# sunnyHelen/JPerceiver

Hardware: AMD Instinct MI355X
Metric: train images/sec (full train step, synthetic 3-frame batches) (higher is better)
Workload: dtype f32

## Files before the change

### include/jperceiver_hip.h

```cpp
#ifndef JPERCEIVER_HIP_H
#define JPERCEIVER_HIP_H
#include <stdint.h>

#ifdef __cplusplus
extern "C" {
#endif

int jp_conv2d_fwd(const float* x, const float* w, const float* bias, float* y, int N, int Cin, int H, int W, int Cout, int KH, int stride, int pad, int pad_mode, int act, float* ws, int ws_state, float* split_ws, const float* amax_x, float* amax_y, int* amax_y_done, float* amax_ws, float* bn_stats, int* bn_stats_parts, void* stream);
int jp_conv2d_fwd_src3(const float* x0, int c0, int up0, const float* x1, int c1, int up1, const float* x2, int c2, int up2, const float* w, const float* bias, float* y, int N, int H, int W, int Cout, int KH, int stride, int pad, int pad_mode, int act, float* ws, int ws_state, float* split_ws, const float* amax_x0, const float* amax_x1, const float* amax_x2, float* amax_y, int* amax_y_done, float* amax_ws, float* bn_stats, int* bn_stats_parts, void* stream);
int jp_conv2d_dgrad(const float* dy, const float* w, float* dx, int N, int Cin, int H, int W, int Cout, int KH, int stride, int pad, int pad_mode, int accumulate, float* ws, int ws_state, float* split_ws, const float* amax_dy, float* amax_dx, int* amax_dx_done, float* amax_ws, void* stream);
int jp_conv2d_dgrad_src3(const float* dy, const float* w, float* dx0, int c0, int up0, int acc0, float* dx1, int c1, int up1, int acc1, float* dx2, int c2, int up2, int acc2, int N, int H, int W, int Cout, int KH, int stride, int pad, int pad_mode, float* ws, int ws_state, float* split_ws, const float* amax_dy, float* amax_dx0, int* amax_dx0_done, float* amax_ws, void* stream);
long jp_conv2d_dgrad_src3_split_floats(int c0, int up0, int c1, int up1, int c2, int up2, int N, int H, int W);
int jp_conv2d_dgrad_src3_ok(int c0, int up0, int c1, int up1, int c2, int up2, int N, int H, int W, int Cout, int KH, int stride, int pad, int pad_mode);
int jp_conv2d_up_head_ok(int c0, int up0, int c1, int c2, int Cout, int KH, int stride, int pad, int pad_mode, int H, int W);
int jp_conv2d_wgrad(const float* x, const float* dy, float* dw, int N, int Cin, int H, int W, int Cout, int KH, int stride, int pad, int pad_mode, int accumulate, float* ws, long ws_floats, const float* amax_x, const float* amax_dy, float* amax_ws, void* stream);
int jp_conv2d_wgrad_src3(const float* x0, int c0, int up0, const float* x1, int c1, int up1, const float* x2, int c2, int up2, const float* dy, float* dw, int N, int H, int W, int Cout, int KH, int stride, int pad, int pad_mode, int accumulate, float* ws, long ws_floats, const float* amax_x0, const float* amax_x1, const float* amax_x2, const float* amax_dy, float* amax_ws, void* stream);
long jp_conv2d_ws_floats(int Cin, int Cout, int KH, int which);
long jp_conv2d_fwd_bn_stats_floats(int N, int OH, int OW, int Cout);
long jp_conv2d_fwd_split_floats(int N, int Cin, int H, int W, int Cout, int KH, int stride, int pad);
long jp_conv2d_dgrad_split_floats(int N, int Cin, int H, int W, int Cout, int KH, int stride, int pad);
long jp_conv2d_wgrad_ws_floats(int N, int Cin, int H, int W, int Cout, int KH, int stride, int pad);
long jp_conv2d_wgrad_src3_ws_floats(int c0, int up0, int c1, int up1, int c2, int up2, int N, int H, int W, int Cout, int KH, int stride, int pad, int pad_mode);
long jp_channel_sum_ws_floats(int N, int C, int HW);
int jp_channel_sum(const float* x, float* out, int N, int C, int HW, int accumulate, float* ws, void* stream);
// ... 12 lines not shown
long jp_bn_ws_doubles(int N, int C, int HW);
int jp_bn_train_fwd(const float* x, const float* gamma, const float* beta, const float* residual, float* y, float* running_mean, float* running_var, float* save_mean, float* save_invstd, double* ws, int N, int C, int HW, float momentum, float eps, int relu, int n_updates, float* amax_y, const float* conv_stats, int conv_parts, void* stream);
int jp_bn_train_bwd(const float* dy, const float* x, const float* y, const float* gamma, const float* beta, const float* save_mean, const float* save_invstd, float* dx, float* dres, float* dgamma, float* dbeta, double* ws, int N, int C, int HW, int relu, int acc_param_grads, float* amax_dx, void* stream);
int jp_bn_eval_fwd(const float* x, const float* gamma, const float* beta, const float* running_mean, const float* running_var, const float* residual, float* y, int N, int C, int HW, float eps, int relu, void* stream);
int jp_bn_relu_pool_fwd(const float* x, const float* gamma, const float* beta, float* pooled, uint8_t* idx, float* running_mean, float* running_var, float* save_mean, float* save_invstd, double* ws, int N, int C, int H, int W, float momentum, float eps, int n_updates, float* amax_y, void* stream);
long jp_bn_relu_pool_bwd_ws_doubles(int N, int C, int H, int W);
int jp_bn_relu_pool_bwd(const float* dpool, const uint8_t* idx, const float* x, const float* gamma, const float* beta, const float* save_mean, const float* save_invstd, float* dx, float* dgamma, float* dbeta, double* ws, int N, int C, int H, int W, int acc_param_grads, void* stream);

int jp_bn_fold_conv(const float* w, const float* conv_bias, const float* gamma, const float* beta, const float* running_mean, const float* running_var, float eps, float* w_out, float* bias_out, int Cout, int K, void* stream);
int jp_add_relu(const float* a, const float* b, float* out, long n, int relu, float* amax_out, void* stream);

int jp_maxpool_fwd(const float* x, float* y, uint8_t* idx, int NC, int H, int W, int k, int s, int p, void* stream);
int jp_maxpool_bwd(const float* dy, const uint8_t* idx, float* dx, const float* addend, int NC, int H, int W, int k, int s, int p, float* amax_dx, void* stream);
int jp_upsample2x_fwd(const float* x, float* y, int N, int C, int H, int W, int dstC, int dc0, void* stream);
int jp_upsample2x_bwd(const float* dy, float* dx, int N, int C, int H, int W, int Ctot, int c0, int accumulate, void* stream);
int jp_copy_channels(const float* src, float* dst, int N, int C, int HW, int srcC, int sc0, int dstC, int dc0, int accumulate, void* stream);
int jp_axpby(const float* a, const float* b, float* out, long n, float alpha, float beta, void* stream);
int jp_sum_n(const float* a0, const float* a1, const float* a2, const float* a3, const float* a4, float* out, long n, float* amax_out, void* stream);
int jp_mul(const float* a, const float* b, float* out, long n, float scale, void* stream);
int jp_affine(const float* a, float* out, long n, float scale, float shift, void* stream);
int jp_act_fwd(const float* x, float* y, long n, int act, void* stream);
int jp_act_bwd(const float* dy, const float* y, float* dx, long n, int act, float* amax_dx, void* stream);
long jp_act_bwd_bias_ws_floats(int N, int C, int HW);
int jp_act_bwd_bias(const float* dy, const float* y, float* dx, float* dbias, int N, int C, int HW, int act, float* amax_dx, float* bias_ws, void* stream);
int jp_mul_bcast_c(const float* a, const float* s, float* out, int N, int C, int HW, void* stream);
int jp_mul_bcast_c_bwd_s(const float* dout, const float* a, float* ds, int N, int C, int HW, void* stream);
int jp_bilinear_fwd(const float* x, float* y, int NC, int H, int W, int OH, int OW, void* stream);
int jp_bilinear_bwd(const float* dy, float* dx, int NC, int H, int W, int OH, int OW, int accumulate, void* stream);
int jp_area_downsample(const float* x, float* y, int NC, int H, int W, int f, void* stream);
int jp_fill(float* out, long n, float v, void* stream);
int jp_warp_perspective(const float* src, const float* Hm, float* dst, int B, int h, int w, int OH, int OW, void* stream);
int jp_softmax_c2(const float* x, float* y, int N, int HW, void* stream);
int jp_disp_to_depth(const float* disp, float* depth, long n, float min_depth, float max_depth, void* stream);
int jp_scale_label_assemble(const float* zwarp, const float* laywarp, const uint8_t* polymask, float* out, int B, int H, int W, int mode, void* stream);
int jp_fill_convex_poly(const int* pts, int npts, uint8_t* mask, int H, int W, void* stream);

int jp_gemm_strided_batched(const float* A, const float* B, float* C, int M, int N, int K, int lda, int ldb, int ldc, long strideA, long strideB, long strideC, int batch, int transA, int transB, float alpha, float beta, void* stream);
int jp_bias_act_rows(float* y, const float* bias, int M, int N, int act, void* stream);
int jp_colsum(const float* x, float* out, int M, int N, int accumulate, void* stream);
int jp_colmax(const float* E, float* val, int64_t* arg, int B, int R, int Cn, void* stream);
int jp_colmax_bwd(const float* dval, const int64_t* arg, float* dE, int B, int R, int Cn, void* stream);
int jp_gather_cols(const float* V, const int64_t* arg, float* T, int B, int C, int Nn, void* stream);
int jp_gather_cols_bwd(const float* dT, const int64_t* arg, float* dV, int B, int C, int Nn, void* stream);
int jp_spatial_mean(const float* x, float* out, int BC, int HW, float scale, void* stream);
int jp_spatial_mean_bwd(const float* dout, float* dx, int BC, int HW, float scale, void* stream);
int jp_bcast_matmul_fwd(const float* attn, const float* V, float* out, int B, int C, int n, void* stream);
int jp_bcast_matmul_bwd(const float* attn, const float* V, const float* dOut, float* dattn, float* dV, int B, int C, int n, void* stream);
int jp_ratio_finalize(const double* acc, float* out, double scale, void* stream);

int jp_pose_fwd(const float* axisangle, const float* translation, const float* K, float* T, float* P, int B, int invert, void* stream);
int jp_pose_bwd(const double* dP, const float* axisangle, const float* translation, const float* K, float* daxisangle, float* dtranslation, int B, int invert, int accumulate, void* stream);
int jp_cgt_warp_fwd(const float* disp, int hs, int ws, const float* invK, const float* P, const float* color, float* pred, int B, int H, int W, float min_depth, float max_depth, void* stream);
int jp_cgt_warp_bwd(const float* dpred, const float* disp, int hs, int ws, const float* invK, const float* P, const float* color, float* ddisp_up, double* dP, int B, int H, int W, float min_depth, float max_depth, int accumulate, void* stream);
int jp_ssim_l1_fwd(const float* pred, const float* target, float* out, int B, int H, int W, void* stream);
int jp_ssim_l1_bwd(const float* pred, const float* target, const int64_t* min_index, int cand, const float* gout, float gscale, float* dpred, int B, int H, int W, void* stream);
int jp_minreproj_fwd(const float* c0, const float* c1, const float* c2, const float* c3, const float* noise0, const float* noise1, int64_t* min_index, double* acc, long total, void* stream);
int jp_scalar_finalize(const double* in, float* out, int n, double scale, void* stream);
int jp_ssim_map(const float* x, const float* y, float* out, int NC, int H, int W, void* stream);
int jp_backproject(const float* depth, const float* invK, float* out, int B, int H, int W, void* stream);
int jp_project(const float* points, const float* K, const float* T, float* out, int B, int H, int W, float eps, void* stream);

int jp_row_sum(const float* x, double* out, int rows, int cols, void* stream);
int jp_smooth_fwd(const float* disp, const double* dsum, const float* img, double* acc, int B, int h, int w, void* stream);
int jp_smooth_bwd(const float* disp, const double* dsum, const float* img, const float* gout, float scale, float* g, double* gd, float* ddisp, int B, int h, int w, int accumulate, void* stream);
int jp_scale_loss_fwd(const float* disp, int hs, int ws, const float* label, double* acc, int B, int FH, int FW, float min_depth, float max_depth, int y_lo, int y_hi, int x_lo, int x_hi, void* stream);
int jp_scale_loss_bwd(const float* disp, int hs, int ws, const float* label, const double* acc, const float* gout, float scale, float* ddisp, int B, int FH, int FW, float min_depth, float max_depth, int y_lo, int y_hi, int x_lo, int x_hi, int accumulate, void* stream);
int jp_layout_loss_fwd(const float* logits, const float* label, const float* sdf, double* sums, float* loss, int B, int h, int w, float w0, float w1, float lw, float cew, float l2w, float ra, float ralpha, float rbeta, void* stream);
int jp_layout_loss_bwd(const float* logits, const float* label, const float* sdf, const double* sums, const float* gout, float* dlogits, int B, int h, int w, float w0, float w1, float lw, float cew, float l2w, float ra, float ralpha, float rbeta, int accumulate, void* stream);
int jp_sdf(const float* label, float* sdf, int* ws, int B, int h, int w, void* stream);
int jp_l1_fwd(const float* a, const float* b, double* acc, long n, void* stream);
int jp_l1_bwd(const float* a, const float* b, const float* gout, float scale, float* da, float* db, long n, void* stream);

int jp_sumsq_blocks(void);
int jp_grad_sumsq_partials(const float* g, double* partials, long n, void* stream);
int jp_sum_doubles(const double* in, double* out, int count, void* stream);
int jp_adam_clip_step(float* p, const float* g, float* m, float* v, long n, const double* normsq, float grad_scale, float max_norm, double lr, double beta1, double beta2, double eps, int step, void* stream);
int jp_adam_clip_step_dev(float* p, const float* g, float* m, float* v, long n, const double* normsq, float grad_scale, float max_norm, double beta1, double beta2, double eps, const float* state, void* stream);
int jp_rng_keep_mask(float* out, long n, uint64_t seed, float p_drop, void* stream);
int jp_rng_normal(float* out, long n, uint64_t seed, void* stream);
int jp_rng_keep_mask_dev(float* out, long n, const long* base, long offset, float p_drop, void* stream);
int jp_rng_normal_dev(float* out, long n, const long* base, long offset, void* stream);

int jp_confusion2(const float* logits, const float* gt, double* counts, int B, int HW, void* stream);
int jp_depth_eval_prepare(const float* disp_resized, const float* gt, float* pred, uint8_t* valid, int H, int W, int y0, int y1, int x0, int x1, float dmin, float dmax, void* stream);
int jp_masked_median(const float* x, const uint8_t* valid, int n, float* out, void* stream);
int jp_depth_errors(const float* gt, const float* pred, const uint8_t* valid, int n, const float* med_gt, const float* med_pred, float fixed_scale, float dmin, float dmax, double* sums, void* stream);

long jp_depth_eval_batch_ws_bytes(int B, int H, int W);
int jp_depth_eval_batch(const float* disp, const float* gt, int B, int h, int w, int H, int W, int y0, int y1, int x0, int x1, float mask_min, float mask_max, double min_depth, double max_depth, float fixed_scale, double* sums, float* med, void* ws, void* stream);
long jp_lidar_depth_ws_bytes(int B, int H, int W);
int jp_lidar_depth_map(const float* pts, const long long* offsets, const double* P, const unsigned char* flip, int B, int H, int W, int vel_depth, double* out64, float* out32, void* ws, void* stream);

int jp_disp_resize_depth(const float* disp, float* depth_out, float* disp_out, int B, int h, int w, int OH, int OW, double min_depth, double max_depth, void* stream);
long jp_quantiles_ws_bytes(int rows);
int jp_quantiles(const float* x, int rows, int n, const float* q, int nq, float* out, void* ws, void* stream);
int jp_colorize_u8(const float* x, int rows, int n, const float* vmin_vmax, const uint8_t* lut, uint8_t* out, void* stream);
int jp_layout_classes_u8(const float* road_logits, const float* car_logits, uint8_t* cls, uint8_t* rgb, int B, int HW, void* stream);

int jp_stream_pose_pair(const float* frame, float* ring, const int* count, float* pair, float* amax_out, int B, int H, int W, void* stream);
int jp_stream_traj_push(const float* T, double* pose, double* traj, int* count, int B, int capacity, void* stream);

int jp_bev_fuse(const uint8_t* layout, const double* pose, int pose_stride, int N, int* counts, int B, int occ, double res_f, double off, double max_range, int Mh, int Mw, double res, double org_r, double org_c, void* stream);
int jp_bev_map_classes(const int* counts, uint8_t* cls, uint8_t* rgb, int B, int cells, double min_seen, double road_frac, double car_frac, void* stream);
int jp_bev_map_mark(uint8_t* rgb, int B, int Mh, int Mw, const double* traj, int n, int capacity, double res, double org_r, double org_c, int color, void* stream);

int jp_depth_bev_lift(const float* depth, const double* cam, int* grid, int B, int H, int W, int occ, double res_f, double off, double min_range, double max_range, double h_min, double h_max, double obst_h, int accumulate, void* stream);
int jp_depth_bev_classes(const int* grid, uint8_t* cls, float* height, int B, int cells, int min_points, int obst_points, void* stream);
int jp_bev_agree(const uint8_t* lifted, const uint8_t* layout, int* out, int B, int cells, void* stream);
// ... 38 lines not shown
```

### jperceiver_amd/csrc/photometric.hip

```cpp
#include "jp_common.h"
#include <algorithm>

namespace {

constexpr int TPB = 256;
constexpr float SSIM_C1 = 0.0001f, SSIM_C2 = 0.0009f;

__device__ void rodrigues(const float v[3], float R[9]) {
    const float th = sqrtf(v[0] * v[0] + v[1] * v[1] + v[2] * v[2]);
    const float inv = 1.f / (th + 1e-7f);
    const float x = v[0] * inv, y = v[1] * inv, z = v[2] * inv;
    const float ca = cosf(th), sa = sinf(th), C = 1.f - ca;
    R[0] = x * x * C + ca;     R[1] = x * y * C - z * sa; R[2] = z * x * C + y * sa;
    R[3] = x * y * C + z * sa; R[4] = y * y * C + ca;     R[5] = y * z * C - x * sa;
    R[6] = z * x * C - y * sa; R[7] = y * z * C + x * sa; R[8] = z * z * C + ca;
}

__global__ void pose_fwd_kernel(const float* __restrict__ aa, const float* __restrict__ tr,
                                const float* __restrict__ K, float* __restrict__ T, float* __restrict__ P, int B,
                                int invert) {
    const int b = blockIdx.x * blockDim.x + threadIdx.x;
    if (b >= B) return;
    float v[3] = {aa[3 * b], aa[3 * b + 1], aa[3 * b + 2]};
    float t[3] = {tr[3 * b], tr[3 * b + 1], tr[3 * b + 2]};
// ... 183 lines not shown
    for (int it = 0; it < CGT_PPT; ++it) {
        const int p = (blockIdx.x * CGT_PPT + it) * TPB + threadIdx.x;
        if (p >= H * W) break;
        const int y = p / W, x = p - y * W;
        const float* Pb = Pm + 12 * b;
        const WarpGeo g = warp_geo(disp + (size_t)b * hs * ws, hs, ws, invK + 16 * b, Pb, y, x, H, W, min_disp,
                                   max_disp, (float)hs / (float)H, (float)ws / (float)W);
        const int x0 = (int)floorf(g.ix), y0 = (int)floorf(g.iy);
        const float tx = g.ix - (float)x0, ty = g.iy - (float)y0;
        const bool xin = x0 + 1 <= W - 1, yin = y0 + 1 <= H - 1;
        const int x1 = xin ? x0 + 1 : x0, y1 = yin ? y0 + 1 : y0;
        const size_t HW = (size_t)H * W;
        const float* c = color + (size_t)b * 3 * HW;
        float gix = 0.f, giy = 0.f;
#pragma unroll
        for (int ch = 0; ch < 3; ++ch) {
            const float* cc = c + ch * HW;
            const float go = dpred[((size_t)b * 3 + ch) * HW + p];
            const float v00 = cc[y0 * W + x0];
            const float v01 = xin ? cc[y0 * W + x1] : 0.f;
            const float v10 = yin ? cc[y1 * W + x0] : 0.f;
            const float v11 = (xin && yin) ? cc[y1 * W + x1] : 0.f;
            gix += go * (-(v00 * (1.f - ty)) + v01 * (1.f - ty) - v10 * ty + v11 * ty);
            giy += go * (-(v00 * (1.f - tx)) - v01 * tx + v10 * (1.f - tx) + v11 * tx);
        }
        const float du = gix * g.mx * (0.5f * (float)W) * (2.f / (float)(W - 1));
        const float dv = giy * g.my * (0.5f * (float)H) * (2.f / (float)(H - 1));
        const float zi = g.pz + 1e-7f;
        const float dpx = du / zi, dpy = dv / zi;
        const float dpz = -(du * g.px + dv * g.py) / (zi * zi);
        const float X = g.depth * g.rx, Y = g.depth * g.ry, Z = g.depth * g.rz;
        dPl[0] += dpx * X; dPl[1] += dpx * Y; dPl[2] += dpx * Z; dPl[3] += dpx;
        dPl[4] += dpy * X; dPl[5] += dpy * Y; dPl[6] += dpy * Z; dPl[7] += dpy;
        dPl[8] += dpz * X; dPl[9] += dpz * Y; dPl[10] += dpz * Z; dPl[11] += dpz;
        const float dX = Pb[0] * dpx + Pb[4] * dpy + Pb[8] * dpz;
        const float dY = Pb[1] * dpx + Pb[5] * dpy + Pb[9] * dpz;
        const float dZ = Pb[2] * dpx + Pb[6] * dpy + Pb[10] * dpz;
        const float ddepth = dX * g.rx + dY * g.ry + dZ * g.rz;
        const float dd = -(max_disp - min_disp) * g.depth * g.depth * ddepth;
        float* q = ddisp_up + (size_t)b * HW + p;
        *q = accumulate ? *q + dd : dd;
    }
    const int lane = threadIdx.x & 63, wv = threadIdx.x >> 6;
#pragma unroll
    for (int i = 0; i < 12; ++i) {
        const float s = jp_wave_sum(dPl[i]);
        if (lane == 0) red[i][wv] = s;
    }
    __syncthreads();
    if (threadIdx.x < 12) {
        const double s = (double)red[threadIdx.x][0] + red[threadIdx.x][1] + red[threadIdx.x][2] + red[threadIdx.x][3];
        atomicAdd(&dP[12 * b + threadIdx.x], s);
    }
}

constexpr int SSIM_ROWS = 4;

struct RowSums { float x, y, xx, yy, xy; };

__device__ __forceinline__ RowSums ssim_hsum(const float* __restrict__ xr, const float* __restrict__ yr, int il, int ic,
                                             int ir, float& xc, float& yc) {
    const float xl = xr[il], xrn = xr[ir], yl = yr[il], yrn = yr[ir];
    xc = xr[ic];
    yc = yr[ic];
    RowSums s;
    s.x = xl + xc + xrn;
    s.y = yl + yc + yrn;
    s.xx = xl * xl + xc * xc + xrn * xrn;
    s.yy = yl * yl + yc * yc + yrn * yrn;
    s.xy = xl * yl + xc * yc + xrn * yrn;
    return s;
}

__global__ __launch_bounds__(TPB) void ssim_l1_fwd_kernel(const float* __restrict__ pred,
                                                          const float* __restrict__ target,
                                                          float* __restrict__ out, int H, int W) {
    const int lane = threadIdx.x & 63, wv = threadIdx.x >> 6;
    const int x = (blockIdx.x * 4 + wv) * 64 + lane;
    if ((blockIdx.x * 4 + wv) * 64 >= W) return;
    const int b = blockIdx.z;
    const int ybeg = blockIdx.y * SSIM_ROWS, yend = min(H, ybeg + SSIM_ROWS);
    const size_t HW = (size_t)H * W;
    const int ic = min(x, W - 1), il = jp_reflect(ic - 1, W), ir = jp_reflect(ic + 1, W);
    float accS[SSIM_ROWS], accL[SSIM_ROWS];
#pragma unroll
    for (int r = 0; r < SSIM_ROWS; ++r) accS[r] = accL[r] = 0.f;
#pragma unroll
    for (int ch = 0; ch < 3; ++ch) {
        const float* xp = pred + ((size_t)b * 3 + ch) * HW;
        const float* yp = target + ((size_t)b * 3 + ch) * HW;
        RowSums r0, r1, r2;
        float xc, yc, xc1, yc1;
        {
            const size_t oa = (size_t)jp_reflect(ybeg - 1, H) * W, ob = (size_t)ybeg * W;
            r0 = ssim_hsum(xp + oa, yp + oa, il, ic, ir, xc, yc);
            r1 = ssim_hsum(xp + ob, yp + ob, il, ic, ir, xc1, yc1);
        }
#pragma unroll
        for (int r = 0; r < SSIM_ROWS; ++r) {
            const int y = min(ybeg + r, H - 1);
            const size_t on = (size_t)jp_reflect(y + 1, H) * W;
            float xc2, yc2;
            r2 = ssim_hsum(xp + on, yp + on, il, ic, ir, xc2, yc2);
            const float k = 1.f / 9.f;
            const float mx = (r0.x + r1.x + r2.x) * k, my = (r0.y + r1.y + r2.y) * k;
            const float sx = (r0.xx + r1.xx + r2.xx) * k - mx * mx;
// ... 63 lines not shown
            const float xl = nxl, xr = nxr, yl = nyl, yr = nyr;
            xc2 = nxc; yc2 = nyc;
            const int miv = nmi;
            if (t + 1 < SSIMB_ROWS + 2) {
                on = rowoff(t + 1);
                nxl = xp[on + il]; nxc = xp[on + ic]; nxr = xp[on + ir];
                nyl = yp[on + il]; nyc = yp[on + ic]; nyr = yp[on + ir];
                if (mi32) nmi = mi32[2 * ((size_t)qrow(t + 1) * W + ic)];
            }
            r2.x = xl + xc2 + xr;
            r2.y = yl + yc2 + yr;
            r2.xx = xl * xl + xc2 * xc2 + xr * xr;
            r2.yy = yl * yl + yc2 * yc2 + yr * yr;
            r2.xy = xl * yl + xc2 * yc2 + xr * yr;
            const bool q_in = q >= 0 && q < H && col_in;
            const float g = (q_in && miv == cand) ? gs : 0.f;
            const float k = 1.f / 9.f;
            const float mx = (r0.x + r1.x + r2.x) * k, my = (r0.y + r1.y + r2.y) * k;
            const float vx = (r0.xx + r1.xx + r2.xx) * k - mx * mx, vy = (r0.yy + r1.yy + r2.yy) * k - my * my;
            const float cxy = (r0.xy + r1.xy + r2.xy) * k - mx * my;
            const float n1 = 2.f * mx * my + SSIM_C1, n2 = 2.f * cxy + SSIM_C2;
            const float d1 = mx * mx + my * my + SSIM_C1, d2 = vx + vy + SSIM_C2;
            const float n = n1 * n2, d = d1 * d2;
            const float invd = 1.f / d, nd = n * invd;
            const float val = (1.f - nd) * 0.5f;
            const float gk = (val >= 0.f && val <= 1.f) ? g * (2.f / 9.f) : 0.f;
            const float G = gk * n1 * invd;
            const float Bc = -gk * nd * d1 * invd;
            const float A = gk * (my * (n2 - n1) * invd - nd * mx * (d2 - d1) * invd);
            const float hA2 = wl * __shfl_up(A, 1, 64) + A + wr * __shfl_down(A, 1, 64);
            const float hB2 = wl * __shfl_up(Bc, 1, 64) + Bc + wr * __shfl_down(Bc, 1, 64);
            const float hG2 = wl * __shfl_up(G, 1, 64) + G + wr * __shfl_down(G, 1, 64);
            if (t >= 2) {
                const int ry = q - 1;
                if (ry < yend && col_out) {
                    const float wu = (ry == 1) ? 2.f : 1.f, wd = (ry == H - 2) ? 2.f : 1.f;
                    const float SA = wu * hA0 + hA1 + wd * hA2;
                    const float SB = wu * hB0 + hB1 + wd * hB2;
                    const float SG = wu * hG0 + hG1 + wd * hG2;
                    const float df = xo - yo;
                    const float l1 = go * df * rsqrtf(df * df + 1e-6f);
                    dp[(size_t)ry * W + cq] = -0.5f * (0.85f / 3.f) * (SA + xo * SB + yo * SG) + (0.15f / 3.f) * l1;
                }
            }
            xo = xc1; yo = yc1; go = g;
            hA0 = hA1; hB0 = hB1; hG0 = hG1;
            hA1 = hA2; hB1 = hB2; hG1 = hG2;
            r0 = r1; r1 = r2;
            xc1 = xc2; yc1 = yc2;
        }
    }
}

__global__ __launch_bounds__(TPB) void minreproj_kernel(const float* __restrict__ c0, const float* __restrict__ c1,
                                                        const float* __restrict__ c2, const float* __restrict__ c3,
                                                        const float* __restrict__ n0, const float* __restrict__ n1,
                                                        int64_t* __restrict__ idx, double* __restrict__ acc,
                                                        long total) {
    __shared__ double sm[4];
    double s = 0.0;
    for (long i = (long)blockIdx.x * TPB + threadIdx.x; i < total; i += (long)gridDim.x * TPB) {
        float best = c0[i] + (n0 ? n0[i] * 1e-5f : 0.f);
        int bi = 0;
        if (c1) { const float v = c1[i] + (n1 ? n1[i] * 1e-5f : 0.f); if (v < best) { best = v; bi = 1; } }
        if (c2) { const float v = c2[i]; if (v < best) { best = v; bi = 2; } }
        if (c3) { const float v = c3[i]; if (v < best) { best = v; bi = 3; } }
        idx[i] = bi;
        s += (double)best;
    }
    s = jp_block_sum_d(s, sm);
    if (threadIdx.x == 0) atomicAdd(acc, s);
}

__global__ void scalar_finalize_kernel(const double* __restrict__ in, float* __restrict__ out, int n,
                                       double scale) {
    const int i = blockIdx.x * blockDim.x + threadIdx.x;
    if (i < n) out[i] = (float)(in[i] * scale);
}

__global__ __launch_bounds__(TPB) void ssim_map_kernel(const float* __restrict__ x, const float* __restrict__ y,
                                                       float* __restrict__ out, long total, int H, int W) {
    for (long i = (long)blockIdx.x * TPB + threadIdx.x; i < total; i += (long)gridDim.x * TPB) {
        const int px = (int)(i % W);
        const long t = i / W;
        const int py = (int)(t % H);
        const long plane = (t / H) * (long)H * W;
        float sx = 0.f, sy = 0.f, sxx = 0.f, syy = 0.f, sxy = 0.f;
#pragma unroll
        for (int dy = -1; dy <= 1; ++dy) {
            const int yy = jp_reflect(py + dy, H);
#pragma unroll
            for (int dx = -1; dx <= 1; ++dx) {
                const int xx = jp_reflect(px + dx, W);
                const float a = x[plane + (long)yy * W + xx], b = y[plane + (long)yy * W + xx];
                sx += a; sy += b; sxx += a * a; syy += b * b; sxy += a * b;
            }
        }
        const float k = 1.f / 9.f;
        const float mx = sx * k, my = sy * k;
        const float vx = sxx * k - mx * mx, vy = syy * k - my * my, cxy = sxy * k - mx * my;
        const float n = (2.f * mx * my + SSIM_C1) * (2.f * cxy + SSIM_C2);
        const float d = (mx * mx + my * my + SSIM_C1) * (vx + vy + SSIM_C2);
        out[i] = fminf(fmaxf((1.f - n / d) * 0.5f, 0.f), 1.f);
    }
}

// ... 31 lines not shown
                P[4 * r + c] = k[4 * r] * t[c] + k[4 * r + 1] * t[4 + c] + k[4 * r + 2] * t[8 + c] + k[4 * r + 3] * t[12 + c];
        const float* q = pts + (long)b * 4 * HW + p;
        const float X = q[0], Y = q[HW], Z = q[2 * HW], Wc = q[3 * HW];
        const float cx = P[0] * X + P[1] * Y + P[2] * Z + P[3] * Wc;
        const float cy = P[4] * X + P[5] * Y + P[6] * Z + P[7] * Wc;
        const float cz = P[8] * X + P[9] * Y + P[10] * Z + P[11] * Wc;
        const float inv = 1.f / (cz + eps);
        out[2 * i] = (cx * inv / (float)(W - 1) - 0.5f) * 2.f;
        out[2 * i + 1] = (cy * inv / (float)(H - 1) - 0.5f) * 2.f;
    }
}

}

#define JP_ST hipStream_t st = (hipStream_t)stream

extern "C" int jp_pose_fwd(const float* axisangle, const float* translation, const float* K, float* T, float* P,
                           int B, int invert, void* stream) {
    JP_CHECK_ARG(axisangle && translation && K && T && P && B > 0, "pose_fwd: bad args");
    JP_ST;
    hipLaunchKernelGGL(pose_fwd_kernel, dim3(jp_cdiv(B, 64)), dim3(64), 0, st, axisangle, translation, K, T, P, B, invert);
    JP_LAUNCH_CHECK();
}

extern "C" int jp_pose_bwd(const double* dP, const float* axisangle, const float* translation, const float* K,
                           float* daxisangle, float* dtranslation, int B, int invert, int accumulate, void* stream) {
    JP_CHECK_ARG(dP && axisangle && translation && K && daxisangle && dtranslation && B > 0, "pose_bwd: bad args");
    JP_ST;
    hipLaunchKernelGGL(pose_bwd_kernel, dim3(jp_cdiv(B, 64)), dim3(64), 0, st, dP, axisangle, translation, K,
                       daxisangle, dtranslation, B, invert, accumulate);
    JP_LAUNCH_CHECK();
}

extern "C" int jp_cgt_warp_fwd(const float* disp, int hs, int ws, const float* invK, const float* P,
                               const float* color, float* pred, int B, int H, int W, float min_depth,
                               float max_depth, void* stream) {
    JP_CHECK_ARG(disp && invK && P && color && pred && B > 0 && H > 1 && W > 1, "cgt_warp_fwd: bad args");
    JP_ST;
    hipLaunchKernelGGL(cgt_warp_fwd_kernel, dim3(jp_cdiv(W, TPB), B, jp_cdiv(H, CGT_FROWS)), dim3(TPB), 0, st, disp, hs, ws, invK, P,
                       color, pred, H, W, 1.f / max_depth, 1.f / min_depth);
    JP_LAUNCH_CHECK();
}

extern "C" int jp_cgt_warp_bwd(const float* dpred, const float* disp, int hs, int ws, const float* invK,
                               const float* P, const float* color, float* ddisp_up, double* dP, int B, int H, int W,
                               float min_depth, float max_depth, int accumulate, void* stream) {
    JP_CHECK_ARG(dpred && disp && invK && P && color && ddisp_up && dP && B > 0, "cgt_warp_bwd: bad args");
    JP_ST;
    hipLaunchKernelGGL(cgt_warp_bwd_kernel, dim3(jp_cdiv((long)H * W, TPB * CGT_PPT), B), dim3(TPB), 0, st, dpred, disp, hs, ws,
                       invK, P, color, ddisp_up, dP, H, W, 1.f / max_depth, 1.f / min_depth, accumulate);
    JP_LAUNCH_CHECK();
}

extern "C" int jp_ssim_l1_fwd(const float* pred, const float* target, float* out, int B, int H, int W,
                              void* stream) {
    JP_CHECK_ARG(pred && target && out && B > 0 && H >= 2 && W >= 2, "ssim_l1_fwd: bad args");
    JP_ST;
    dim3 grid(jp_cdiv(W, 256), jp_cdiv(H, SSIM_ROWS), B);
    hipLaunchKernelGGL(ssim_l1_fwd_kernel, grid, dim3(TPB), 0, st, pred, target, out, H, W);
    JP_LAUNCH_CHECK();
}

extern "C" int jp_ssim_l1_bwd(const float* pred, const float* target, const int64_t* min_index, int cand,
                              const float* gout, float gscale, float* dpred, int B, int H, int W, void* stream) {
    JP_CHECK_ARG(pred && target && dpred && B > 0 && H >= 2 && W >= 2, "ssim_l1_bwd: bad args");
    JP_ST;
    dim3 grid(jp_cdiv(jp_cdiv(W, 62), 4), jp_cdiv(H, SSIMB_ROWS), B);
    hipLaunchKernelGGL(ssim_l1_bwd_kernel, grid, dim3(TPB), 0, st, pred, target, min_index, cand, gout, gscale, dpred,
                       H, W);
    JP_LAUNCH_CHECK();
}

extern "C" int jp_minreproj_fwd(const float* c0, const float* c1, const float* c2, const float* c3,
                                const float* noise0, const float* noise1, int64_t* min_index, double* acc,
                                long total, void* stream) {
    JP_CHECK_ARG(c0 && min_index && acc && total > 0, "minreproj_fwd: bad args");
    JP_ST;
    JP_HIP(hipMemsetAsync(acc, 0, sizeof(double), st));
    hipLaunchKernelGGL(minreproj_kernel, dim3((int)std::min<long>((total + TPB - 1) / TPB, 2048)), dim3(TPB), 0, st,
                       c0, c1, c2, c3, noise0, noise1, min_index, acc, total);
    JP_LAUNCH_CHECK();
}

extern "C" int jp_scalar_finalize(const double* in, float* out, int n, double scale, void* stream) {
    JP_CHECK_ARG(in && out && n > 0, "scalar_finalize: bad args");
    JP_ST;
    hipLaunchKernelGGL(scalar_finalize_kernel, dim3(jp_cdiv(n, 64)), dim3(64), 0, st, in, out, n, scale);
    JP_LAUNCH_CHECK();
}

extern "C" int jp_ssim_map(const float* x, const float* y, float* out, int NC, int H, int W, void* stream) {
    JP_CHECK_ARG(x && y && out && NC > 0 && H >= 2 && W >= 2, "ssim_map: bad args");
    JP_ST;
    const long total = (long)NC * H * W;
    hipLaunchKernelGGL(ssim_map_kernel, dim3((int)std::min<long>((total + TPB - 1) / TPB, 65535)), dim3(TPB), 0, st, x, y, out,
                       total, H, W);
    JP_LAUNCH_CHECK();
}

extern "C" int jp_backproject(const float* depth, const float* invK, float* out, int B, int H, int W, void* stream) {
    JP_CHECK_ARG(depth && invK && out && B > 0 && H > 0 && W > 0, "backproject: bad args");
    JP_ST;
    const long total = (long)B * H * W;
    hipLaunchKernelGGL(backproject_kernel, dim3((int)std::min<long>((total + TPB - 1) / TPB, 65535)), dim3(TPB), 0, st, depth,
                       invK, out, B, H, W);
    JP_LAUNCH_CHECK();
// ... 12 lines not shown
```

### jperceiver_amd/ops_loss.py

```python
from __future__ import annotations

import torch

from ._lib import call
from . import ops
from .ops import Var, _rec, _new, gemm


def bmm_tn(k: Var, q: Var) -> Var:
    B, C, N = k.t.shape
    e = _new((B, N, N), k.t)
    gemm(k.t, q.t, e, N, N, C, N, N, N, C * N, C * N, N * N, B, tA=1)
    out = Var(e, k.rg or q.rg)

    def bwd():
        if out.g is None:
            return
        dE = out.g
        if k.rg:
            g, acc = k.grad_buf()
            gemm(q.t, dE, g, C, N, N, N, N, N, C * N, N * N, C * N, B, tB=1, beta=float(acc))
        if q.rg:
            g, acc = q.grad_buf()
            gemm(k.t, dE, g, C, N, N, N, N, N, C * N, N * N, C * N, B, beta=float(acc))
        out.g = None

    _rec(out.rg, bwd)
    return out


def colmax(e: Var, want_arg=True):
    B, R, N = e.t.shape
    val = _new((B, N), e.t)
    arg = _new((B, N), e.t, torch.int64)
    call("jp_colmax", e.t, val, arg, B, R, N)
    out = Var(val, e.rg)

    def bwd():
        if out.g is None:
            return
        d = torch.empty_like(e.t)
        call("jp_colmax_bwd", out.g, arg, d, B, R, N)
        e.add_grad(d)
        out.g = None

    _rec(out.rg, bwd)
    return out, arg


def gather_cols(v: Var, arg: torch.Tensor) -> Var:
    B, C, N = v.t.shape
    t = torch.empty_like(v.t)
    call("jp_gather_cols", v.t, arg, t, B, C, N)
# ... 83 lines not shown
        self.vals = torch.zeros(len(self.names), device=device, dtype=torch.float32)
        self.grads = torch.zeros(len(self.names), device=device, dtype=torch.float32)

    def val(self, name):
        i = self.index[name]
        return self.vals[i:i + 1]

    def grad(self, name):
        i = self.index[name]
        return self.grads[i:i + 1]


def combine(lv: LossVec, out_name, terms):
    o = lv.val(out_name)
    first = True
    for name, c in terms:
        call("jp_axpby", lv.val(name), None if first else o, o, 1, float(c), 1.0)
        first = False

    def bwd():
        go = lv.grad(out_name)
        for name, c in terms:
            g = lv.grad(name)
            call("jp_axpby", go, g, g, 1, float(c), 1.0)

    _rec(True, bwd)


class PoseP:
    __slots__ = ("T", "P", "dP")

    def __init__(self, T, P, dP):
        self.T, self.P, self.dP = T, P, dP


def pose(axisangle: Var, translation: Var, K: torch.Tensor, invert: bool) -> PoseP:
    B = axisangle.t.shape[0]
    T = _new((B, 4, 4), K)
    P = _new((B, 3, 4), K)
    call("jp_pose_fwd", axisangle.t, translation.t, K, T, P, B, int(invert))
    dP = torch.zeros((B, 12), device=K.device, dtype=torch.float64) if (axisangle.rg or translation.rg) else None
    pp = PoseP(T, P, dP)

    def bwd():
        ga, acc = axisangle.grad_buf()
        gt, acc2 = translation.grad_buf()
        assert acc == acc2
        call("jp_pose_bwd", dP, axisangle.t, translation.t, K, ga, gt, B, int(invert), acc)

    _rec(dP is not None, bwd)
    return pp


def ssim_l1(pred: torch.Tensor, target: torch.Tensor) -> torch.Tensor:
    B, _, H, W = pred.shape
    out = _new((B, 1, H, W), pred)
    call("jp_ssim_l1_fwd", pred, target, out, B, H, W)
    return out


def min_reprojection_loss(lv: LossVec, slot, disp: Var, poses, colors, target, invK, id_losses, noises,
                          H, W, min_depth, max_depth, n_scales):
    B = disp.t.shape[0]
    hs, ws = disp.t.shape[2], disp.t.shape[3]
    preds, rls = [], []
    for pp, col in zip(poses, colors):
        pred = _new((B, 3, H, W), target)
        call("jp_cgt_warp_fwd", disp.t, hs, ws, invK, pp.P, col, pred, B, H, W, min_depth, max_depth)
        preds.append(pred)
        rls.append(ssim_l1(pred, target))
    cands = list(id_losses) + rls
    assert 1 <= len(cands) <= 4 and len(id_losses) <= 2
    c = cands + [None] * (4 - len(cands))
    nz = list(noises) + [None] * (2 - len(noises))
    idx = _new((B, H, W), target, torch.int64)
    acc = _new((1,), target, torch.float64)
    total = B * H * W
    call("jp_minreproj_fwd", c[0], c[1], c[2], c[3], nz[0], nz[1], idx, acc, total)
    gscale = 1.0 / (total * n_scales)
    call("jp_scalar_finalize", acc, lv.val(slot), 1, gscale)

    def bwd():
        gout = lv.grad(slot)
        dup = None
        for j, (pp, col, pred) in enumerate(zip(poses, colors, preds)):
            need_pose = pp.dP is not None
            if not (disp.rg or need_pose):
                continue
            dpred = torch.empty_like(pred)
            call("jp_ssim_l1_bwd", pred, target, idx, len(id_losses) + j, gout, gscale, dpred, B, H, W)
            first = dup is None
            if first:
                dup = _new((B, 1, H, W), target)
            dP = pp.dP if need_pose else torch.zeros((B, 12), device=target.device, dtype=torch.float64)
            call("jp_cgt_warp_bwd", dpred, disp.t, hs, ws, invK, pp.P, col, dup, dP, B, H, W, min_depth, max_depth,
                 0 if first else 1)
        if disp.rg and dup is not None:
            g, acc_ = disp.grad_buf()
            call("jp_bilinear_bwd", dup, g, B, hs, ws, H, W, acc_)

    _rec(True, bwd)
    return preds, idx


def scale_loss(lv: LossVec, slot, disp: Var, label: torch.Tensor, weight, min_depth, max_depth, crop=None):
    B, _, hs, ws = disp.t.shape
    FH, FW = label.shape[2], label.shape[3]
    y0, y1, x0, x1 = crop if crop is not None else (0, FH, 0, FW)
    acc = _new((2,), disp.t, torch.float64)
    call("jp_scale_loss_fwd", disp.t, hs, ws, label, acc, B, FH, FW, min_depth, max_depth, y0, y1, x0, x1)
    call("jp_ratio_finalize", acc, lv.val(slot), float(weight))

    def bwd():
        if not disp.rg:
            return
        g, a = disp.grad_buf()
        call("jp_scale_loss_bwd", disp.t, hs, ws, label, acc, lv.grad(slot), float(weight), g, B, FH, FW, min_depth,
             max_depth, y0, y1, x0, x1, a)

    _rec(True, bwd)


def smooth_loss(lv: LossVec, slot, disp: Var, img_ds: torch.Tensor, weight):
    B, _, h, w = disp.t.shape
    dsum = _new((B,), disp.t, torch.float64)
    call("jp_row_sum", disp.t, dsum, B, h * w)
    acc = _new((1,), disp.t, torch.float64)
    call("jp_smooth_fwd", disp.t, dsum, img_ds, acc, B, h, w)
    call("jp_scalar_finalize", acc, lv.val(slot), 1, float(weight))

    def bwd():
        if not disp.rg:
            return
        g = torch.empty_like(disp.t)
        gd = _new((B,), disp.t, torch.float64)
        dd, a = disp.grad_buf()
        call("jp_smooth_bwd", disp.t, dsum, img_ds, lv.grad(slot), float(weight), g, gd, dd, B, h, w, a)

    _rec(True, bwd)


def signed_distance(label: torch.Tensor) -> torch.Tensor:
    B, _, h, w = label.shape
    sdf = _new((B, h, w), label)
    ws = _new((2 * B * h * w + B,), label, torch.int32)
    call("jp_sdf", label, sdf, ws, B, h, w)
    return sdf
# ... 43 lines not shown
```

Before: 123.8.

## Save warp sampling gradients in forward and fuse SSIM-L1 backward with warp backward

The warp forward kernel now also stores the per-channel bilinear sampling gradients (6 channels per pixel) during the forward pass. A new fused backward kernel computes the SSIM+L1 gradient w.r.t. the predicted image and immediately contracts it with the saved coefficients, then runs the geometric backward tail for disparity and pose. This removes the intermediate dpred tensor and the separate warp backward kernel, including its re-gather of source colors. In exchange it writes and keeps a B×6×H×W buffer per source frame, adds shared-memory staging, and repeats per-block dP atomics.

```diff
diff --git a/include/jperceiver_hip.h b/include/jperceiver_hip.h
--- a/include/jperceiver_hip.h
+++ b/include/jperceiver_hip.h
@@ -88,8 +88,11 @@
 int jp_pose_bwd(const double* dP, const float* axisangle, const float* translation, const float* K, float* daxisangle, float* dtranslation, int B, int invert, int accumulate, void* stream);
 int jp_cgt_warp_fwd(const float* disp, int hs, int ws, const float* invK, const float* P, const float* color, float* pred, int B, int H, int W, float min_depth, float max_depth, void* stream);
 int jp_cgt_warp_bwd(const float* dpred, const float* disp, int hs, int ws, const float* invK, const float* P, const float* color, float* ddisp_up, double* dP, int B, int H, int W, float min_depth, float max_depth, int accumulate, void* stream);
+int jp_cgt_warp_fwd_save(const float* disp, int hs, int ws, const float* invK, const float* P, const float* color, float* pred, float* coef, int B, int H, int W, float min_depth, float max_depth, void* stream);
+int jp_cgt_warp_bwd_coef(const float* dpred, const float* coef, const float* disp, int hs, int ws, const float* invK, const float* P, float* ddisp_up, double* dP, int B, int H, int W, float min_depth, float max_depth, int accumulate, void* stream);
 int jp_ssim_l1_fwd(const float* pred, const float* target, float* out, int B, int H, int W, void* stream);
 int jp_ssim_l1_bwd(const float* pred, const float* target, const int64_t* min_index, int cand, const float* gout, float gscale, float* dpred, int B, int H, int W, void* stream);
+int jp_ssim_l1_warp_bwd(const float* pred, const float* target, const int64_t* min_index, int cand, const float* gout, float gscale, const float* coef, const float* disp, int hs, int ws, const float* invK, const float* P, float* ddisp_up, double* dP, int B, int H, int W, float min_depth, float max_depth, int accumulate, void* stream);
 int jp_minreproj_fwd(const float* c0, const float* c1, const float* c2, const float* c3, const float* noise0, const float* noise1, int64_t* min_index, double* acc, long total, void* stream);
 int jp_scalar_finalize(const double* in, float* out, int n, double scale, void* stream);
 int jp_ssim_map(const float* x, const float* y, float* out, int NC, int H, int W, void* stream);
diff --git a/jperceiver_amd/csrc/photometric.hip b/jperceiver_amd/csrc/photometric.hip
--- a/jperceiver_amd/csrc/photometric.hip
+++ b/jperceiver_amd/csrc/photometric.hip
@@ -259,6 +259,119 @@
         const double s = (double)red[threadIdx.x][0] + red[threadIdx.x][1] + red[threadIdx.x][2] + red[threadIdx.x][3];
         atomicAdd(&dP[12 * b + threadIdx.x], s);
     }
+}
+
+
+__device__ __forceinline__ void warp_sample_grad(float v00, float v01, float v10, float v11, bool xin, bool yin, float tx,
+                                                 float ty, float& gx, float& gy) {
+    if (!xin) v01 = 0.f;
+    if (!yin) v10 = 0.f;
+    if (!(xin && yin)) v11 = 0.f;
+    gx = -(v00 * (1.f - ty)) + v01 * (1.f - ty) - v10 * ty + v11 * ty;
+    gy = -(v00 * (1.f - tx)) - v01 * tx + v10 * (1.f - tx) + v11 * tx;
+}
+
+__global__ __launch_bounds__(TPB) void cgt_warp_fwd_save_kernel(const float* __restrict__ disp, int hs, int ws,
+                                                                const float* __restrict__ invK,
+                                                                const float* __restrict__ Pm,
+                                                                const float* __restrict__ color,
+                                                                float* __restrict__ pred, float* __restrict__ coef, int H,
+                                                                int W, float min_disp, float max_disp) {
+    const int b = blockIdx.y;
+    const int x = blockIdx.x * TPB + threadIdx.x;
+    if (x >= W) return;
+    const size_t HW = (size_t)H * W;
+    const float* c = color + (size_t)b * 3 * HW;
+#pragma unroll
+    for (int it = 0; it < CGT_FROWS; ++it) {
+        const int y = blockIdx.z * CGT_FROWS + it;
+        if (y >= H) break;
+        const int p = y * W + x;
+        const WarpGeo g = warp_geo(disp + (size_t)b * hs * ws, hs, ws, invK + 16 * b, Pm + 12 * b, y, x, H, W, min_disp,
+                                   max_disp, (float)hs / (float)H, (float)ws / (float)W);
+        const int x0 = (int)floorf(g.ix), y0 = (int)floorf(g.iy);
+        const float tx = g.ix - (float)x0, ty = g.iy - (float)y0;
+        const bool xin = x0 + 1 <= W - 1, yin = y0 + 1 <= H - 1;
+        const int x1 = min(x0 + 1, W - 1), y1 = min(y0 + 1, H - 1);
+        const float w00 = (1.f - tx) * (1.f - ty), w01 = tx * (1.f - ty), w10 = (1.f - tx) * ty, w11 = tx * ty;
+#pragma unroll
+        for (int ch = 0; ch < 3; ++ch) {
+            const float* cc = c + ch * HW;
+            const float v00 = cc[y0 * W + x0], v01 = cc[y0 * W + x1], v10 = cc[y1 * W + x0], v11 = cc[y1 * W + x1];
+            pred[((size_t)b * 3 + ch) * HW + p] = v00 * w00 + v01 * w01 + v10 * w10 + v11 * w11;
+            float gx, gy;
+            warp_sample_grad(v00, v01, v10, v11, xin, yin, tx, ty, gx, gy);
+            coef[((size_t)b * 6 + ch) * HW + p] = gx;
+            coef[((size_t)b * 6 + 3 + ch) * HW + p] = gy;
+        }
+    }
+}
+
+__device__ __forceinline__ float warp_bwd_tail(const WarpGeo& g, float gix, float giy, const float* __restrict__ Pb, int H, int W,
+                                               float min_disp, float max_disp, float (&dPl)[12]) {
+    const float du = gix * g.mx * (0.5f * (float)W) * (2.f / (float)(W - 1));
+    const float dv = giy * g.my * (0.5f * (float)H) * (2.f / (float)(H - 1));
+    const float zi = g.pz + 1e-7f;
+    const float dpx = du / zi, dpy = dv / zi;
+    const float dpz = -(du * g.px + dv * g.py) / (zi * zi);
+    const float X = g.depth * g.rx, Y = g.depth * g.ry, Z = g.depth * g.rz;
+    dPl[0] += dpx * X; dPl[1] += dpx * Y; dPl[2] += dpx * Z; dPl[3] += dpx;
+    dPl[4] += dpy * X; dPl[5] += dpy * Y; dPl[6] += dpy * Z; dPl[7] += dpy;
+    dPl[8] += dpz * X; dPl[9] += dpz * Y; dPl[10] += dpz * Z; dPl[11] += dpz;
+    const float dX = Pb[0] * dpx + Pb[4] * dpy + Pb[8] * dpz;
+    const float dY = Pb[1] * dpx + Pb[5] * dpy + Pb[9] * dpz;
+    const float dZ = Pb[2] * dpx + Pb[6] * dpy + Pb[10] * dpz;
+    const float ddepth = dX * g.rx + dY * g.ry + dZ * g.rz;
+    return -(max_disp - min_disp) * g.depth * g.depth * ddepth;
+}
+
+__device__ __forceinline__ void warp_dP_reduce(const float (&dPl)[12], float (*red)[4], double* __restrict__ dPb) {
+    const int lane = threadIdx.x & 63, wv = threadIdx.x >> 6;
+#pragma unroll
+    for (int i = 0; i < 12; ++i) {
+        const float s = jp_wave_sum(dPl[i]);
+        if (lane == 0) red[i][wv] = s;
+    }
+    __syncthreads();
+    if (threadIdx.x < 12) {
+        const double s = (double)red[threadIdx.x][0] + red[threadIdx.x][1] + red[threadIdx.x][2] + red[threadIdx.x][3];
+        atomicAdd(&dPb[threadIdx.x], s);
+    }
+}
+
+__global__ __launch_bounds__(TPB) void cgt_warp_bwd_coef_kernel(const float* __restrict__ dpred,
+                                                                const float* __restrict__ coef,
+                                                                const float* __restrict__ disp, int hs, int ws,
+                                                                const float* __restrict__ invK,
+                                                                const float* __restrict__ Pm,
+                                                                float* __restrict__ ddisp_up, double* __restrict__ dP,
+                                                                int H, int W, float min_disp, float max_disp,
+                                                                int accumulate) {
+    __shared__ float red[12][4];
+    const int b = blockIdx.y;
+    const size_t HW = (size_t)H * W;
+    const float* Pb = Pm + 12 * b;
+    float dPl[12];
+#pragma unroll
+    for (int i = 0; i < 12; ++i) dPl[i] = 0.f;
+    for (int it = 0; it < CGT_PPT; ++it) {
+        const int p = (blockIdx.x * CGT_PPT + it) * TPB + threadIdx.x;
+        if (p >= H * W) break;
+        const int y = p / W, x = p - y * W;
+        float gix = 0.f, giy = 0.f;
+#pragma unroll
+        for (int ch = 0; ch < 3; ++ch) {
+            const float go = dpred[((size_t)b * 3 + ch) * HW + p];
+            gix += go * coef[((size_t)b * 6 + ch) * HW + p];
+            giy += go * coef[((size_t)b * 6 + 3 + ch) * HW + p];
+        }
+        const WarpGeo g = warp_geo(disp + (size_t)b * hs * ws, hs, ws, invK + 16 * b, Pb, y, x, H, W, min_disp,
+                                   max_disp, (float)hs / (float)H, (float)ws / (float)W);
+        const float dd = warp_bwd_tail(g, gix, giy, Pb, H, W, min_disp, max_disp, dPl);
+        float* q = ddisp_up + (size_t)b * HW + p;
+        *q = accumulate ? *q + dd : dd;
+    }
+    warp_dP_reduce(dPl, red, dP + 12 * b);
 }
 
 constexpr int SSIM_ROWS = 4;
@@ -428,6 +541,140 @@
     }
 }
 
+__global__ __launch_bounds__(TPB) void ssim_l1_warp_bwd_kernel(const float* __restrict__ pred,
+                                                               const float* __restrict__ target,
+                                                               const int64_t* __restrict__ min_index, int cand,
+                                                               const float* __restrict__ gout, float gscale,
+                                                               const float* __restrict__ coef,
+                                                               const float* __restrict__ disp, int hs, int ws,
+                                                               const float* __restrict__ invK,
+                                                               const float* __restrict__ Pm,
+                                                               float* __restrict__ ddisp_up, double* __restrict__ dP, int H,
+                                                               int W, float min_disp, float max_disp, int accumulate) {
+    __shared__ float sg[SSIMB_ROWS][2][TPB];
+    __shared__ float red[12][4];
+    const int lane = threadIdx.x & 63, wv = threadIdx.x >> 6;
+    const int strip = blockIdx.x * 4 + wv;
+    const bool strip_in = strip * 62 < W;
+    const int cq = strip * 62 - 1 + lane;
+    const bool col_in = strip_in && cq >= 0 && cq < W;
+    const bool col_out = col_in && lane >= 1 && lane <= 62;
+    const int ic = min(max(cq, 0), W - 1), il = jp_reflect(ic - 1, W), ir = jp_reflect(ic + 1, W);
+    const float wl = (cq == 1) ? 2.f : 1.f, wr = (cq == W - 2) ? 2.f : 1.f;
+    const int b = blockIdx.z;
+    const int ybeg = blockIdx.y * SSIMB_ROWS, yend = min(H, ybeg + SSIMB_ROWS);
+    const size_t HW = (size_t)H * W;
+    if (strip_in) {
+        const float gs = gscale * (gout ? gout[0] : 1.f);
+        const int* mi32 = min_index ? reinterpret_cast<const int*>(min_index + (size_t)b * HW) : nullptr;
+#pragma unroll 1
+        for (int ch = 0; ch < 3; ++ch) {
+            const float* xp = pred + ((size_t)b * 3 + ch) * HW;
+            const float* yp = target + ((size_t)b * 3 + ch) * HW;
+            const float* cx = coef + ((size_t)b * 6 + ch) * HW;
+            RowSums r0, r1, r2;
+            float xc1, yc1, xc2, yc2;
+            {
+                float xd, yd;
+                const size_t oa = (size_t)jp_reflect(min(max(ybeg - 2, -1), H), H) * W;
+                const size_t ob = (size_t)jp_reflect(ybeg - 1, H) * W;
+                r0 = ssim_hsum(xp + oa, yp + oa, il, ic, ir, xd, yd);
+                r1 = ssim_hsum(xp + ob, yp + ob, il, ic, ir, xc1, yc1);
+            }
+            float hA0 = 0.f, hB0 = 0.f, hG0 = 0.f, hA1 = 0.f, hB1 = 0.f, hG1 = 0.f;
+            float xo = 0.f, yo = 0.f, go = 0.f;
+            auto rowoff = [&](int t) -> size_t { return (size_t)jp_reflect(min(ybeg + t, H), H) * W; };
+            auto qrow = [&](int t) -> int { return min(max(ybeg - 1 + t, 0), H - 1); };
+            auto crow = [&](int t) -> size_t { return (size_t)min(ybeg + max(t - 2, 0), H - 1) * W; };
+            size_t on = rowoff(0);
+            float nxl = xp[on + il], nxc = xp[on + ic], nxr = xp[on + ir], nyl = yp[on + il], nyc = yp[on + ic], nyr = yp[on + ir];
+            int nmi = mi32 ? mi32[2 * ((size_t)qrow(0) * W + ic)] : cand;
+            float ncx = 0.f, ncy = 0.f;
+#pragma unroll 1
+            for (int t = 0; t < SSIMB_ROWS + 2; ++t) {
+                const int q = ybeg - 1 + t;
+                const float xl = nxl, xr = nxr, yl = nyl, yr = nyr;
+                xc2 = nxc; yc2 = nyc;
+                const int miv = nmi;
+                const float cfx = ncx, cfy = ncy;
+                if (t + 1 < SSIMB_ROWS + 2) {
+                    on = rowoff(t + 1);
+                    nxl = xp[on + il]; nxc = xp[on + ic]; nxr = xp[on + ir];
+                    nyl = yp[on + il]; nyc = yp[on + ic]; nyr = yp[on + ir];
+                    if (mi32) nmi = mi32[2 * ((size_t)qrow(t + 1) * W + ic)];
+                    if (t + 1 >= 2) {
+                        const size_t oc = crow(t + 1) + ic;
+                        ncx = cx[oc]; ncy = cx[3 * HW + oc];
+                    }
+                }
+                r2.x = xl + xc2 + xr;
+                r2.y = yl + yc2 + yr;
+                r2.xx = xl * xl + xc2 * xc2 + xr * xr;
+                r2.yy = yl * yl + yc2 * yc2 + yr * yr;
+                r2.xy = xl * yl + xc2 * yc2 + xr * yr;
+                const bool q_in = q >= 0 && q < H && col_in;
+                const float g = (q_in && miv == cand) ? gs : 0.f;
+                const float k = 1.f / 9.f;
+                const float mx = (r0.x + r1.x + r2.x) * k, my = (r0.y + r1.y + r2.y) * k;
+                const float vx = (r0.xx + r1.xx + r2.xx) * k - mx * mx, vy = (r0.yy + r1.yy + r2.yy) * k - my * my;
+                const float cxy = (r0.xy + r1.xy + r2.xy) * k - mx * my;
+                const float n1 = 2.f * mx * my + SSIM_C1, n2 = 2.f * cxy + SSIM_C2;
+                const float d1 = mx * mx + my * my + SSIM_C1, d2 = vx + vy + SSIM_C2;
+                const float n = n1 * n2, d = d1 * d2;
+                const float invd = 1.f / d, nd = n * invd;
+                const float val = (1.f - nd) * 0.5f;
+                const float gk = (val >= 0.f && val <= 1.f) ? g * (2.f / 9.f) : 0.f;
+                const float G = gk * n1 * invd;
+                const float Bc = -gk * nd * d1 * invd;
+                const float A = gk * (my * (n2 - n1) * invd - nd * mx * (d2 - d1) * invd);
+                const float hA2 = wl * __shfl_up(A, 1, 64) + A + wr * __shfl_down(A, 1, 64);
+                const float hB2 = wl * __shfl_up(Bc, 1, 64) + Bc + wr * __shfl_down(Bc, 1, 64);
+                const float hG2 = wl * __shfl_up(G, 1, 64) + G + wr * __shfl_down(G, 1, 64);
+                if (t >= 2) {
+                    const int ry = q - 1;
+                    if (ry < yend && col_out) {
+                        const float wu = (ry == 1) ? 2.f : 1.f, wd = (ry == H - 2) ? 2.f : 1.f;
+                        const float SA = wu * hA0 + hA1 + wd * hA2;
+                        const float SB = wu * hB0 + hB1 + wd * hB2;
+                        const float SG = wu * hG0 + hG1 + wd * hG2;
+                        const float df = xo - yo;
+                        const float l1 = go * df * rsqrtf(df * df + 1e-6f);
+                        const float dpv = -0.5f * (0.85f / 3.f) * (SA + xo * SB + yo * SG) + (0.15f / 3.f) * l1;
+                        float* s0 = &sg[t - 2][0][threadIdx.x];
+                        float* s1 = &sg[t - 2][1][threadIdx.x];
+                        if (ch == 0) {
+                            *s0 = dpv * cfx; *s1 = dpv * cfy;
+                        } else {
+                            *s0 += dpv * cfx; *s1 += dpv * cfy;
+                        }
+                    }
+                }
+                xo = xc1; yo = yc1; go = g;
+                hA0 = hA1; hB0 = hB1; hG0 = hG1;
+                hA1 = hA2; hB1 = hB2; hG1 = hG2;
+                r0 = r1; r1 = r2;
+                xc1 = xc2; yc1 = yc2;
+            }
+        }
+    }
+    float dPl[12];
+#pragma unroll
+    for (int i = 0; i < 12; ++i) dPl[i] = 0.f;
+    if (col_out) {
+        const float* Pb = Pm + 12 * b;
+#pragma unroll 1
+        for (int r = 0; r < yend - ybeg; ++r) {
+            const int ry = ybeg + r;
+            const WarpGeo g = warp_geo(disp + (size_t)b * hs * ws, hs, ws, invK + 16 * b, Pb, ry, cq, H, W, min_disp, max_disp,
+                                       (float)hs / (float)H, (float)ws / (float)W);
+            const float dd = warp_bwd_tail(g, sg[r][0][threadIdx.x], sg[r][1][threadIdx.x], Pb, H, W, min_disp, max_disp, dPl);
+            float* q = ddisp_up + (size_t)b * HW + (size_t)ry * W + cq;
+            *q = accumulate ? *q + dd : dd;
+        }
+    }
+    warp_dP_reduce(dPl, red, dP + 12 * b);
+}
+
 __global__ __launch_bounds__(TPB) void minreproj_kernel(const float* __restrict__ c0, const float* __restrict__ c1,
                                                         const float* __restrict__ c2, const float* __restrict__ c3,
                                                         const float* __restrict__ n0, const float* __restrict__ n1,
@@ -565,6 +812,41 @@
     JP_LAUNCH_CHECK();
 }
 
+extern "C" int jp_cgt_warp_fwd_save(const float* disp, int hs, int ws, const float* invK, const float* P,
+                                    const float* color, float* pred, float* coef, int B, int H, int W, float min_depth,
+                                    float max_depth, void* stream) {
+    JP_CHECK_ARG(disp && invK && P && color && pred && coef && B > 0 && H > 1 && W > 1 && hs > 0 && ws > 0,
+                 "cgt_warp_fwd_save: bad args");
+    JP_ST;
+    hipLaunchKernelGGL(cgt_warp_fwd_save_kernel, dim3(jp_cdiv(W, TPB), B, jp_cdiv(H, CGT_FROWS)), dim3(TPB), 0, st, disp, hs, ws,
+                       invK, P, color, pred, coef, H, W, 1.f / max_depth, 1.f / min_depth);
+    JP_LAUNCH_CHECK();
+}
+
+extern "C" int jp_cgt_warp_bwd_coef(const float* dpred, const float* coef, const float* disp, int hs, int ws,
+                                    const float* invK, const float* P, float* ddisp_up, double* dP, int B, int H, int W,
+                                    float min_depth, float max_depth, int accumulate, void* stream) {
+    JP_CHECK_ARG(dpred && coef && disp && invK && P && ddisp_up && dP && B > 0 && H > 1 && W > 1 && hs > 0 && ws > 0,
+                 "cgt_warp_bwd_coef: bad args");
+    JP_ST;
+    hipLaunchKernelGGL(cgt_warp_bwd_coef_kernel, dim3(jp_cdiv((long)H * W, TPB * CGT_PPT), B), dim3(TPB), 0, st, dpred, coef, disp,
+                       hs, ws, invK, P, ddisp_up, dP, H, W, 1.f / max_depth, 1.f / min_depth, accumulate);
+    JP_LAUNCH_CHECK();
+}
+
+extern "C" int jp_ssim_l1_warp_bwd(const float* pred, const float* target, const int64_t* min_index, int cand,
+                                   const float* gout, float gscale, const float* coef, const float* disp, int hs, int ws,
+                                   const float* invK, const float* P, float* ddisp_up, double* dP, int B, int H, int W,
+                                   float min_depth, float max_depth, int accumulate, void* stream) {
+    JP_CHECK_ARG(pred && target && coef && disp && invK && P && ddisp_up && dP && B > 0 && H >= 2 && W >= 2 && hs > 0 && ws > 0,
+                 "ssim_l1_warp_bwd: bad args");
+    JP_ST;
+    dim3 grid(jp_cdiv(jp_cdiv(W, 62), 4), jp_cdiv(H, SSIMB_ROWS), B);
+    hipLaunchKernelGGL(ssim_l1_warp_bwd_kernel, grid, dim3(TPB), 0, st, pred, target, min_index, cand, gout, gscale, coef, disp, hs,
+                       ws, invK, P, ddisp_up, dP, H, W, 1.f / max_depth, 1.f / min_depth, accumulate);
+    JP_LAUNCH_CHECK();
+}
+
 extern "C" int jp_ssim_l1_fwd(const float* pred, const float* target, float* out, int B, int H, int W,
                               void* stream) {
     JP_CHECK_ARG(pred && target && out && B > 0 && H >= 2 && W >= 2, "ssim_l1_fwd: bad args");
diff --git a/jperceiver_amd/ops_loss.py b/jperceiver_amd/ops_loss.py
--- a/jperceiver_amd/ops_loss.py
+++ b/jperceiver_amd/ops_loss.py
@@ -1,4 +1,6 @@
 from __future__ import annotations
+
+import os
 
 import torch
 
@@ -188,6 +190,9 @@
     return pp
 
 
+_PHOTO_COEF = os.environ.get("JP_PHOTO_COEF", "1") != "0"
+
+
 def ssim_l1(pred: torch.Tensor, target: torch.Tensor) -> torch.Tensor:
     B, _, H, W = pred.shape
     out = _new((B, 1, H, W), pred)
@@ -199,11 +204,17 @@
                           H, W, min_depth, max_depth, n_scales):
     B = disp.t.shape[0]
     hs, ws = disp.t.shape[2], disp.t.shape[3]
-    preds, rls = [], []
+    preds, rls, coefs = [], [], []
     for pp, col in zip(poses, colors):
         pred = _new((B, 3, H, W), target)
-        call("jp_cgt_warp_fwd", disp.t, hs, ws, invK, pp.P, col, pred, B, H, W, min_depth, max_depth)
+        save = _PHOTO_COEF and ops.current_tape() is not None and (disp.rg or pp.dP is not None)
+        coef = _new((B, 6, H, W), target) if save else None
+        if save:
+            call("jp_cgt_warp_fwd_save", disp.t, hs, ws, invK, pp.P, col, pred, coef, B, H, W, min_depth, max_depth)
+        else:
+            call("jp_cgt_warp_fwd", disp.t, hs, ws, invK, pp.P, col, pred, B, H, W, min_depth, max_depth)
         preds.append(pred)
+        coefs.append(coef)
         rls.append(ssim_l1(pred, target))
     cands = list(id_losses) + rls
     assert 1 <= len(cands) <= 4 and len(id_losses) <= 2
@@ -223,12 +234,17 @@
             need_pose = pp.dP is not None
             if not (disp.rg or need_pose):
                 continue
-            dpred = torch.empty_like(pred)
-            call("jp_ssim_l1_bwd", pred, target, idx, len(id_losses) + j, gout, gscale, dpred, B, H, W)
             first = dup is None
             if first:
                 dup = _new((B, 1, H, W), target)
             dP = pp.dP if need_pose else torch.zeros((B, 12), device=target.device, dtype=torch.float64)
+            if coefs[j] is not None:
+                call("jp_ssim_l1_warp_bwd", pred, target, idx, len(id_losses) + j, gout, gscale, coefs[j], disp.t, hs, ws, invK,
+                     pp.P, dup, dP, B, H, W, min_depth, max_depth, 0 if first else 1)
+                coefs[j] = None
+                continue
+            dpred = torch.empty_like(pred)
+            call("jp_ssim_l1_bwd", pred, target, idx, len(id_losses) + j, gout, gscale, dpred, B, H, W)
             call("jp_cgt_warp_bwd", dpred, disp.t, hs, ws, invK, pp.P, col, dup, dP, B, H, W, min_depth, max_depth,
                  0 if first else 1)
         if disp.rg and dup is not None:
```

Result: no change. 123.1 (-0.5%).
